# caki35/UNet-Torch

Measured on AMD Instinct MI355X. Metric: images/sec training step, 4-level U-Net 1ch→2cls 512×512, at 1/2/4/8 MI355X, higher is better.
Workload: dtype f16

## Files before the change

include/unetmi.h:

```cpp
#ifndef UNETMI_H
#define UNETMI_H
#include <stddef.h>
#include <stdint.h>

#ifdef __cplusplus
extern "C" {
#endif

typedef void* umi_stream_t;

enum { UMI_F32 = 0, UMI_F16 = 1 };
enum { UMI_OK = 0, UMI_ERR_BADARG = -1, UMI_ERR_UNSUPPORTED = -2, UMI_ERR_WORKSPACE = -3 };
enum { UMI_CONV_UPSAMPLE2 = 1,
       UMI_CONV_FORCE_GENERIC = 2,
       UMI_CONV_DGRAD_STRIDED = 4,
       UMI_CONV_ACCUMULATE = 8      };

int umi_version(void);
const char* umi_arch(void);

int umi_tune_conv3x3_impl(int impl);

int umi_pack_kn(const float* src, void* dst, int T, int K, int N, long st, long sk, long sn,
                int flip_t, int Kpad, int Npad, int dtype, umi_stream_t stream);

int umi_pack_kn8(const float* src, void* dst, int T, int K, int N, long st, long sk, long sn,
                 int flip_t, int Kpad, int Npad, int dtype, umi_stream_t stream);

int umi_conv_fwd(const void* x, int ldx, const void* tx, const void* wp, const float* bias,
                 void* y, int ldy, float* stat_part,
                 int N, int H, int W, int Ci, int Co, int R, int S, int stride, int pad,
                 int Ho, int Wo, int off_h, int off_w, int out_H, int out_W,
                 int in_dtype, int out_dtype, int flags, umi_stream_t stream);
int umi_linear_fused(const void* x, int ldx, const void* wp8, const float* bias, void* y, int ldy, long M, int Ci, int Co,
                     int epi, float p, unsigned seed, const unsigned* seed_dev, void* mask, const void* aux, int ldaux,
                     void* y2, int ldy2, int dtype, umi_stream_t stream);

int umi_conv_fwd_plan(int N, int H, int W, int Ci, int Co, int R, int S, int stride, int pad,
                      int ldx, int ldy, int in_dtype, int out_dtype, int flags, int has_bias,
                      int* layout, int* stat_rows);

int umi_bn_finalize(const float* stat_part, int rows, int C, double count,
                    const float* gamma, const float* beta, float eps, float momentum,
                    float* running_mean, float* running_var,
                    void* tx_out, float* rstd_out, umi_stream_t stream);

int umi_pool2_fwd(const void* x, int ldx, const void* tx, void* y, int ldy,
                  int N, int H, int W, int C, int dtype, umi_stream_t stream);
int umi_pool2_bwd(const void* dpool, int lddp, const void* x, int ldx, const void* tx,
                  void* da, int ldda, int accumulate,
                  int N, int H, int W, int C, int dtype, umi_stream_t stream);

size_t umi_bn_bwd_ws_bytes(long M, int C);
int umi_bn_bwd_reduce(const void* da, int ldda, const void* y, int ldy, const void* tx,
                      const float* rstd, float* sum_dz, float* sum_dzx,
                      long M, int C, int dtype, void* ws, size_t ws_bytes, umi_stream_t stream);
int umi_bn_bwd_apply(void* da, int ldda, const void* y, int ldy, const void* tx,
                     const float* rstd, const float* sum_dz, const float* sum_dzx,
                     long M, int C, int dtype, umi_stream_t stream);

int umi_conv_dgrad_bnred(const void* dy, int lddy, const void* wp8, void* da, int ldda, const void* ybn, int ldybn,
                         const void* txbn, const float* rstd, float* part, int N, int H, int W, int Ci, int Co,
                         int dtype, umi_stream_t stream);

int umi_conv_gather_bnred_rows(int N, int H, int W, int Ci, int Co, int R, int S, int stride, int pad, int Ho, int Wo,
                               int ldx, int ldy, int dtype, int flags);
int umi_conv_gather_bnred(const void* x, int ldx, const void* wp8, void* y, int ldy, const void* ybn, int ldybn,
                          const void* txbn, const float* rstd, float* part, int N, int H, int W, int Ci, int Co, int R, int S,
                          int stride, int pad, int Ho, int Wo, int dtype, int flags, umi_stream_t stream);

int umi_head_dgrad_bnred_rows(long P, int Ci, int Co, int ldda, int dtype);
int umi_head_dgrad_bnred(const void* dl, int lddl, const void* wp, void* da, int ldda, const void* ybn, int ldybn,
                         const void* txbn, const float* rstd, float* part, long P, int Ci, int Co, int dtype,
                         umi_stream_t stream);
size_t umi_head_bwd_fused_ws_bytes(long P, int Ci, int Co);
int umi_head_bwd_fused(const void* dl, int lddl, const void* wp, void* da, int ldda, const void* ybn, int ldybn,
                       const void* txbn, const float* rstd, float* part, float* dW, long s_co, long s_ci, float out_scale,
                       void* ws, size_t ws_bytes, long P, int Ci, int Co, int dtype, umi_stream_t stream);

int umi_conv3x3_fwd_act(const void* x, int ldx, const void* tx, const void* wp8, const void* out_tx, void* y, int ldy,
                        int N, int H, int W, int Ci, int Co, int dtype, umi_stream_t stream);
int umi_bn_stats_rows(long M, int C);
int umi_bn_stats(const void* x, int ldx, float* part, long M, int C, int dtype, umi_stream_t stream);
int umi_pool2_bwd_bnred_stat_rows(int N, int H, int W, int C);
int umi_pool2_bwd_bnred(const void* dpool, int lddp, const void* x, int ldx, const void* tx, const float* rstd, void* da,
                        int ldda, int accumulate, float* part, int N, int H, int W, int C, int dtype, umi_stream_t stream);
int umi_bn_bwd_from_partials(const float* part, int rows, int C, float* sum_dz, float* sum_dzx, umi_stream_t stream);

size_t umi_conv_wgrad_ws_bytes(int N, int Ho, int Wo, int Ci, int Co, int R, int S, int dtype, int flags);
int umi_conv_wgrad(const void* x, int ldx, const void* txa, const void* dy, int lddy, const void* txb,
                   float* dW, long s_co, long s_ci, long s_t, float out_scale,
                   int N, int H, int W, int Ci, int Co, int R, int S, int stride, int pad,
                   int Ho, int Wo, int dtype, int flags, void* ws, size_t ws_bytes, umi_stream_t stream);
typedef struct umi_wgrad_pending {
    const float* part;
    float* dW;
    long s_co, s_ci, s_t;
    float scale;
    int splits, RS, Ci, Co;
} umi_wgrad_pending;
int umi_conv_wgrad_deferred(const void* x, int ldx, const void* txa, const void* dy, int lddy, const void* txb,
                            float* dW, long s_co, long s_ci, long s_t, float out_scale, int N, int H, int W, int Ci, int Co,
                            int R, int S, int stride, int pad, int Ho, int Wo, int dtype, int flags, void* ws, size_t ws_bytes,
                            umi_wgrad_pending* out, umi_stream_t stream);
int umi_wgrad_reduce_group(int n, const void* items , umi_stream_t stream);
int umi_conv_wgrad_bias(const void* x, int ldx, const void* dy, int lddy, const void* txb, float* dW, long s_co, long s_ci,
                        long s_t, float* dbias, float out_scale, int N, int H, int W, int Ci, int Co, int Ho, int Wo, int dtype,
                        int flags, void* ws, size_t ws_bytes, umi_wgrad_pending* out, umi_stream_t stream);
int umi_conv_wgrad_group(int n, const void* const* x, int ldx, const void* const* dy, int lddy, float* const* dW, long s_co,
                         long s_ci, float out_scale, long M, int Ci, int Co, int dtype, umi_stream_t stream);
int umi_conv_wgrad_bnapply(const void* x, int ldx, const void* txa, const void* da, int ldda, const void* y, int ldy,
                           const void* tx_bn, const float* rstd, const float* sum_dz, const float* sum_dzx, void* dz,
                           int lddz, float* dW, long s_co, long s_ci, long s_t, float out_scale, int N, int H, int W,
                           int Ci, int Co, int R, int S, int stride, int pad, int dtype, int flags, void* ws,
                           size_t ws_bytes, umi_stream_t stream);

size_t umi_colsum_ws_bytes(long M, int C);
int umi_colsum(const void* x, int ldx, float* out, float out_scale, long M, int C, int dtype,
               void* ws, size_t ws_bytes, umi_stream_t stream);
int umi_colsum_group(int n, const void* const* xs, int ldx, float* const* outs, float out_scale, long M, int C, int dtype,
                     void* ws, size_t ws_bytes, umi_stream_t stream);

int umi_materialize_nchw(const void* x, int ldx, const void* tx, float* y_nchw,
                         int N, int H, int W, int C, int dtype, umi_stream_t stream);


int umi_wstd_fwd(const float* w, float* wstd, float* rstd, int Co, int K, float eps, umi_stream_t stream);
int umi_wstd_bwd(const float* wstd, const float* rstd, const float* g, float* dw, int Co, int K, umi_stream_t stream);
typedef struct umi_wstd_desc {
    const float* w;
    float* ws;
    float* rstd;
    long off;
    int Co, K;
    float eps;
    int blk0;
    float* dw;
} umi_wstd_desc;
int umi_wstd_fwd_multi(const void* descs, int n_desc, int total_rows, umi_stream_t stream);
int umi_wstd_bwd_multi(const void* descs, int n_desc, int total_rows, const float* g_base, float* dw_base, umi_stream_t stream);

size_t umi_gn_fwd_ws_bytes(int N, long HW, int C);
int umi_gn_fwd(const void* x, int ldx, const float* gamma, const float* beta, const void* res, int ldr, void* y, int ldy,
               float* mean, float* rstd, int relu, int N, long HW, int C, int G, float eps, int dtype,
               void* ws, size_t ws_bytes, umi_stream_t stream);
size_t umi_gn_bwd_ws_bytes(int N, long HW, int C, int G);
int umi_gn_bwd(const void* dy, int lddy, const void* y, int ldy, const void* x, int ldx, const float* mean,
               const float* rstd, const float* gamma, int relu, void* dx, int lddx, void* dres, int lddr,
               float* dgamma, float* dbeta, float out_scale, int N, long HW, int C, int G, int dtype,
               void* ws, size_t ws_bytes, float* part_out, umi_stream_t stream);
int umi_gn_param_grads_group(int n, const float* const* parts, const int* Cs, int N, float* const* dgammas,
                             float* const* dbetas, float out_scale, umi_stream_t stream);

int umi_pool3s2_fwd(const void* x, int ldx, void* y, int ldy, void* idx, int N, int H, int W, int C, int dtype,
                    umi_stream_t stream);
int umi_pool3s2_bwd(const void* dy, int lddy, const void* x, int ldx, const void* idx, void* dx, int lddx, int N, int H, int W,
                    int C, int dtype, umi_stream_t stream);

int umi_ln_fwd(const void* x, int ldx, const float* gamma, const float* beta, void* y, int ldy, float* mean, float* rstd,
               long M, int C, float eps, int dtype, umi_stream_t stream);
size_t umi_ln_bwd_ws_bytes(long M, int C);
int umi_ln_bwd(const void* dy, int lddy, const void* x, int ldx, const float* gamma, const float* mean,
               const float* rstd, void* dx, int lddx, float* dgamma, float* dbeta, float out_scale, long M, int C,
               int dtype, void* ws, size_t ws_bytes, int* rows_out, umi_stream_t stream);

int umi_elementwise(int mode, const void* x, int ldx, const void* g, int ldg, void* y, int ldy, long M, int C,
                    long bcast_rows, int dtype, umi_stream_t stream);

int umi_dropout(const void* x, int ldx, void* y, int ldy, void* mask, int backward, float p, unsigned seed, long M, int C,
                int dtype, const void* tx, const unsigned* seed_dev, umi_stream_t stream);
int umi_dropout_fused(const void* x, int ldx, void* y, int ldy, void* mask, int backward, float p, unsigned seed, long M, int C,
                      int dtype, const unsigned* seed_dev, const void* aux, int ldaux, int gelu, umi_stream_t stream);

int umi_attn_fwd(const void* q, const void* k, const void* v, int ld, void* o, int ldo, float* lse, int B, int N, int heads,
                 int D, int dtype, umi_stream_t stream);
int umi_attn_bwd(const void* q, const void* k, const void* v, int ld, const void* o, const void* dO, int ldo,
                 const float* lse, void* dq, void* dk, void* dv, int ldd, float* delta, int B, int N, int heads, int D,
                 int dtype, umi_stream_t stream);

int umi_bilinear2x(const void* x, int ldx, const void* tx, void* y, int ldy, int backward, int N, int H, int W, int C,
                   int dtype, umi_stream_t stream);

size_t umi_dice_ce_ws_bytes(int N, int C, long HW);
int umi_dice_ce_fwd(const float* logits, const void* target, int target_dtype, int N, int C, long HW, float* stats, void* ws,
                    size_t ws_bytes, umi_stream_t stream);
int umi_dice_ce_bwd(const float* logits, const void* target, int target_dtype, const float* stats, const float* gout, int N,
                    int C, long HW, float* dlogits, umi_stream_t stream);

size_t umi_hdt_ws_bytes(int B, int H, int W);
int umi_hdt_fwd(const float* pred, const float* target, int B, int C, int H, int W, float alpha, float* D, float* fields,
                float* loss, void* ws, size_t ws_bytes, umi_stream_t stream);
int umi_hdt_bwd(const float* pred, const float* target, const float* D, const float* gout, int B, int C, int H, int W,
                float* dpred, umi_stream_t stream);

size_t umi_binloss_ws_bytes(int B, int C, long HW);
int umi_dice_bce_fwd(const float* pred, const float* target, int B, long HW, double* stats, float* loss, void* ws,
                     size_t ws_bytes, umi_stream_t stream);
int umi_dice_bce_bwd(const float* pred, const float* target, const double* stats, const float* gout, int B, long HW,
                     float* dpred, umi_stream_t stream);
int umi_tversky_fwd(const float* pred, const void* target, int target_dtype, int B, int C, long HW, float alpha, float beta,
                    double* stats, float* loss, void* ws, size_t ws_bytes, umi_stream_t stream);
int umi_tversky_bwd(const float* pred, const void* target, int target_dtype, const double* stats, const float* gout, int B,
                    int C, long HW, float alpha, float beta, float* dpred, umi_stream_t stream);

size_t umi_topk_loss_ws_bytes(long N);
int umi_topk_loss_fwd(const float* pred, const float* target, long N, long k, int mode, unsigned char* mask, float* loss,
                      void* ws, size_t ws_bytes, umi_stream_t stream);
int umi_topk_loss_bwd(const float* pred, const float* target, const unsigned char* mask, const float* gout, long N, long k,
                      float* dpred, umi_stream_t stream);

size_t umi_mt_ratio_ws_bytes(int B, long HW);
size_t umi_mt_ratio_stats_len(int B);
int umi_mt_ratio_fwd(const float* o1, const float* o2, const float* l1, const float* l2, int B, long HW, int gate,
                     const float* gate_dev, double* stats, float* loss, float* loss1, float* loss2, float* ratio, void* ws, size_t ws_bytes,
                     umi_stream_t stream);
int umi_mt_ratio_bwd(const float* o1, const float* o2, const float* l1, const float* l2, const double* stats,
                     const float* gout, int B, long HW, float* d1, float* d2, umi_stream_t stream);

typedef struct umi_optim_desc {
    float* p;
    const float* g;
    float* s0;
// ... 95 lines not shown
```

unet-torch_amd/csrc/conv1x1_mfma.hip:

```cpp
#include "common.h"
#include <stdlib.h>
#include <string.h>

typedef _Float16 half8 __attribute__((ext_vector_type(8)));
typedef _Float16 half4 __attribute__((ext_vector_type(4)));
typedef float floatx16 __attribute__((ext_vector_type(16)));
typedef float floatx4 __attribute__((ext_vector_type(4)));
typedef unsigned u32x4 __attribute__((ext_vector_type(4)));

struct UmiLinearEpi { int mode; float p; unsigned seed; const unsigned* seed_dev; void* mask; const void* aux; int ldaux; void* y2; int ldy2;
                      const void* bn_tx; const float* bn_rstd; float* bn_part; };

namespace {

constexpr int OUT_UPS_TAPS_MAX = 49;

constexpr int CK = 64;
constexpr int ROWB = 160;

struct Geo {
    int h, w;
    int Hs, Ws, soy, sox;
    int Hd, Wd, doy, dox;
    int S, stride, pad, frac;
// ... 268 lines not shown
            tdx = (tap & 1) + geo.dox;
        }
        constexpr int NPS = P / PSTEP;
        half8 ybv[NPS];
        if (geo.epi == 3 && !OUT_UPS) {
#pragma unroll
            for (int k = 0; k < NPS; ++k) {
                const int p = p0 + k * PSTEP;
                if (m0 + p < M && col_ok) {
                    const int2 pi = dense ? make_int2(0, 0) : pixinfo[p];
                    const long drow = dense ? (m0 + p) : ((long)pi.x * geo.Hd + (pi.y >> 16)) * geo.Wd + (pi.y & 0xffff);
                    ybv[k] = *reinterpret_cast<const half8*>(geo.aux + drow * geo.ldaux + cop);
                }
            }
        }
#pragma unroll
        for (int k = 0; k < NPS; ++k) {
            const int p = p0 + k * PSTEP;
            if (m0 + p >= M || !col_ok) break;
            const int2 pi = dense ? make_int2(0, 0) : pixinfo[p];
            int yy = pi.y >> 16, xx = pi.y & 0xffff;
            if (OUT_UPS) {
                yy = 2 * yy + tdy;
                xx = 2 * xx + tdx;
                if (yy < 0 || yy >= geo.Hd || xx < 0 || xx >= geo.Wd) continue;
            }
            uint4 v = *reinterpret_cast<const uint4*>(smem + p * ERS + j * 16);
            half_t* dst = dense ? y + (m0 + p) * ldy + co : y + ((long)((long)pi.x * geo.Hd + yy) * geo.Wd + xx) * ldy + co;
            if (geo.accum) {
                const half8 o = *reinterpret_cast<const half8*>(dst);
                v = __builtin_bit_cast(uint4, (half8)(o + __builtin_bit_cast(half8, v)));
            }
            if (geo.epi == 1 || geo.epi == 2) {
                const long e0 = (m0 + p) * (long)Ntot_ + cop;
                const unsigned seed = geo.seed + (geo.seed_dev ? geo.seed_dev[0] * 0x9E3779B9u : 0u);
                const float scale = 1.f / (1.f - geo.drop_p);
                const half8 xv = __builtin_bit_cast(half8, v);
                half8 av, o;
                if (geo.epi == 2) av = *reinterpret_cast<const half8*>(geo.aux + (m0 + p) * geo.ldaux + cop);
                unsigned long long mk = 0;
#pragma unroll
                for (int jj = 0; jj < 8; ++jj) {
                    const long e = e0 + jj;
                    const float u = (c1_hash32((unsigned)e, seed ^ (unsigned)(e >> 32)) >> 8) * (1.f / 16777216.f);
                    const unsigned k = u >= geo.drop_p;
                    mk |= (unsigned long long)k << (8 * jj);
                    float f = (float)xv[jj];
                    if (geo.epi == 1) f = c1_gelu(f);
                    f = k ? f * scale : 0.f;
                    if (geo.epi == 2) f += (float)av[jj];
                    o[jj] = (half_t)f;
                }
                *reinterpret_cast<unsigned long long*>(geo.mask + e0) = mk;
                if (geo.epi == 1) *reinterpret_cast<half8*>(geo.y2 + (m0 + p) * geo.ldy2 + cop) = o;
                else v = __builtin_bit_cast(uint4, o);
            }
#ifdef UMI_X_NOSTORE
            if (v.x == 0x12345678u)
#endif
            *reinterpret_cast<uint4*>(dst) = v;
            if (geo.epi == 3 && !OUT_UPS) {
                const half8 yv = ybv[k];
                const half8 hv = __builtin_bit_cast(half8, v);
#pragma unroll
                for (int jj = 0; jj < 8; ++jj) {
                    const float yy_ = (float)yv[jj];
                    const float dz = umi_tx_pre(yy_, bt[jj]) > bt[jj].w ? (float)hv[jj] : 0.f;
                    bs[jj] += dz;
                    bq[jj] = fmaf(dz, (yy_ - bt[jj].x) * brs[jj], bq[jj]);
                }
            }
        }
        if (geo.epi == 3) {
            __syncthreads();
            float* rs_ = reinterpret_cast<float*>(smem);
#pragma unroll
            for (int jj = 0; jj < 8; ++jj) {
                rs_[(0 * PSTEP + p0) * BN + j * 8 + jj] = bs[jj];
                rs_[(1 * PSTEP + p0) * BN + j * 8 + jj] = bq[jj];
            }
            __syncthreads();
            if (tid < 2 * BN) {
                const int which = tid / BN, cc = tid % BN;
                float a = 0.f;
#pragma unroll 8
                for (int k = 0; k < PSTEP; ++k) a += rs_[(which * PSTEP + k) * BN + cc];
                if (c0 + cc < Ntot_) geo.bn_part[((m0 / P) * 2 + which) * Ntot_ + c0 + cc] = a;
            }
        }
    }
}

template <int P, int BN>
int launch(bool s2d, bool ups, const void* x, int ldx, const void* tx, const void* wp8, const float* bias, void* y,
           int ldy, long M, int Kc, int Nc, int Ntot, int ntaps, Geo geo, hipStream_t s) {
    const int n_co = (Ntot + BN - 1) / BN;
    const long nblk = ((M + P - 1) / P) * n_co;
    dim3 grid((unsigned)((nblk + 7) / 8 * 8)), block(256);
#define GO(S2D, UPS, HT)                                                                                          \
    hipLaunchKernelGGL((conv1x1_mfma_kernel<P, BN, S2D, UPS, HT>), grid, block, 0, s, (const half_t*)x, ldx,      \
                       (const float4*)tx, (const half_t*)wp8, bias, (half_t*)y, ldy, M, Kc, Nc, n_co, ntaps, geo, nblk)
    if (s2d) { if (tx) GO(true, false, true); else GO(true, false, false); }
    else if (ups) { if (tx) GO(false, true, true); else GO(false, true, false); }
    else { if (tx) GO(false, false, true); else GO(false, false, false); }
#undef GO
    UMI_LAUNCH_CHECK();
    return UMI_OK;
}

}

int umi_conv1x1_mode(int R, int S, int stride, int pad, int flags) {
    if (flags & UMI_CONV_UPSAMPLE2) return (R == 2 && S == 2) ? 1 : -1;
    if (R * S > 49 || pad < 0 || pad >= 1 << 20) return -1;
    if (flags & UMI_CONV_DGRAD_STRIDED) return stride >= 1 ? 2 : -1;
    if (R == 1 && S == 1 && stride == 1 && pad == 0) return 0;
    if (stride >= 2) return 2;
    return -1;
}

bool umi_conv1x1_mfma_ok(int Ci, int Co, int R, int S, int stride, int pad, int ldx, int ldy, int in_dtype,
                         int out_dtype, int flags) {
    if (flags & UMI_CONV_FORCE_GENERIC) return false;
    if (in_dtype != UMI_F16 || out_dtype != UMI_F16) return false;
    const int mode = umi_conv1x1_mode(R, S, stride, pad, flags);
    if (mode < 0) return false;
    if (ldx % 8 || ldy % 8) return false;
    if ((long)(OUT_UPS_TAPS_MAX) * Ci * Co * 2 >= 0x7FFFFFF0L) return false;
    if (mode == 0) return Ci % 8 == 0 && Co % 8 == 0 && Ci >= 16 && Co >= 16;
    if (Ci % 64 || Co % 64) return false;
    return true;
}

static void c1_pick_tile(long M, int Ntot, int* P, int* BN) {
    const bool bn128 = Ntot % 128 == 0;
    const long want = 300;
    const long b_256_128 = ((M + 255) / 256) * (Ntot / 128), b_128_128 = ((M + 127) / 128) * (Ntot / 128);
    const long b_256_64 = ((M + 255) / 256) * (Ntot / 64);
    if (const char* e = getenv("UMI_C1_TILE")) {
        const int p_ = atoi(e), bn_ = strchr(e, 'x') ? atoi(strchr(e, 'x') + 1) : 0;
        if ((p_ == 256 || p_ == 128) && ((bn_ == 128 && bn128) || bn_ == 64)) { *P = p_; *BN = bn_; return; }
    }
    if (bn128 && b_256_128 >= want) { *P = 256; *BN = 128; return; }
    if (b_256_64 >= want) { *P = 256; *BN = 64; return; }
    if (bn128 && b_128_128 >= want) { *P = 128; *BN = 128; return; }
    *P = 128; *BN = 64;
}
int umi_conv1x1_bnred_rows(long M, int Ntot) {
    int P, BN;
    c1_pick_tile(M, Ntot, &P, &BN);
    return (int)((M + P - 1) / P);
}

int umi_conv1x1_mfma(const void* x, int ldx, const void* tx, const void* wp8, const float* bias, void* y, int ldy,
                     int N, int H, int W, int Ci, int Co, int R, int S, int stride, int pad, int Ho, int Wo, int off_h,
                     int off_w, int out_H, int out_W, int flags, hipStream_t s, const UmiLinearEpi* epi) {
    const int mode = umi_conv1x1_mode(R, S, stride, pad, flags);
    if (epi && epi->mode && epi->mode != 3 && (mode != 0 || (flags & UMI_CONV_ACCUMULATE) || Co % 8)) return UMI_ERR_UNSUPPORTED;
    if (epi && epi->mode == 3 && (mode == 1 || Co % 8)) return UMI_ERR_UNSUPPORTED;
    Geo geo;
    long M;
    int Kc = Ci, Nc = Co, Ntot = Co, ntaps = 1;
    if (mode == 0) {
        geo = Geo{H, W, H, W, 0, 0, H, W, 0, 0, 1, 1, 0, 0};
        M = (long)N * H * W;
    } else if (mode == 1) {
        geo = Geo{H, W, H, W, 0, 0, out_H, out_W, off_h, off_w, 1, 1, 0, 0};
        M = (long)N * H * W;
        Ntot = 4 * Co;
    } else {
        geo = Geo{Ho, Wo, H, W, 0, 0, Ho, Wo, 0, 0, S, stride, pad, (flags & UMI_CONV_DGRAD_STRIDED) ? 1 : 0};
        M = (long)N * Ho * Wo;
        ntaps = R * S;
    }
    if (mode != 0 && 2L * H * W * ldx * 2 >= 0x7FFFFFF0L) return UMI_ERR_UNSUPPORTED;
    geo.accum = (flags & UMI_CONV_ACCUMULATE) ? 1 : 0;
    geo.epi = 0; geo.drop_p = 0.f; geo.seed = 0; geo.seed_dev = nullptr; geo.mask = nullptr; geo.aux = nullptr; geo.ldaux = 0;
    geo.y2 = nullptr; geo.ldy2 = 0; geo.bn_tx = nullptr; geo.bn_rstd = nullptr; geo.bn_part = nullptr;
    if (epi && epi->mode) {
        geo.epi = epi->mode; geo.drop_p = epi->p; geo.seed = epi->seed; geo.seed_dev = epi->seed_dev;
        geo.mask = (unsigned char*)epi->mask; geo.aux = (const half_t*)epi->aux; geo.ldaux = epi->ldaux;
        geo.y2 = (half_t*)epi->y2; geo.ldy2 = epi->ldy2;
        geo.bn_tx = (const float4*)epi->bn_tx; geo.bn_rstd = epi->bn_rstd; geo.bn_part = epi->bn_part;
    }
#define GO(P_, BN_) return launch<P_, BN_>(mode == 2, mode == 1, x, ldx, tx, wp8, bias, y, ldy, M, Kc, Nc, Ntot, ntaps, geo, s)
    int tp, tbn;
    c1_pick_tile(M, Ntot, &tp, &tbn);
    if (tp == 256 && tbn == 128) GO(256, 128);
    if (tp == 256) GO(256, 64);
    if (tbn == 128) GO(128, 128);
    GO(128, 64);
#undef GO
}
```

unet-torch_amd/umi/lib.py:

```python
import ctypes
import os
from ctypes import c_char_p, c_double, c_float, c_int, c_long, c_size_t, c_uint, c_void_p

from . import build as _build

UMI_F32, UMI_F16 = 0, 1
CONV_UPSAMPLE2, CONV_FORCE_GENERIC, CONV_DGRAD_STRIDED, CONV_ACCUMULATE = 1, 2, 4, 8

_ERR = {-1: "UMI_ERR_BADARG", -2: "UMI_ERR_UNSUPPORTED", -3: "UMI_ERR_WORKSPACE"}


def _load():
    alt = os.environ.get("UMI_LIB_OVERRIDE")
    if alt:
        if not os.path.exists(alt):
            raise RuntimeError(f"UMI_LIB_OVERRIDE={alt} does not exist")
        return ctypes.CDLL(alt)
    path = _build.LIB
    if not os.path.exists(path) or (_build.stale() and os.path.exists(_build.HIPCC)):
        if not os.path.exists(_build.HIPCC):
            raise RuntimeError(
                f"libunetmi.so not found at {path} and hipcc is unavailable: the HIP extension is "
                "required, there is no CPU fallback (run `python __graft_entry__.py build`).")
        _build.build_lib()
    return ctypes.CDLL(path)


_lib = _load()

SIGNATURES = {
    "umi_version": (c_int, []),
    "umi_arch": (c_char_p, []),
    "umi_tune_conv3x3_impl": (c_int, [c_int]),
    "umi_zoom_cubic_ws_bytes": (c_size_t, [c_int, c_int, c_int]),
    "umi_zoom_cubic_hwc": (c_int, [c_void_p, c_int, c_void_p, c_int, c_int, c_int, c_int, c_int, c_void_p, c_size_t, c_void_p]),
    "umi_linear_fused": (c_int, [c_void_p, c_int, c_void_p, c_void_p, c_void_p, c_int, c_long, c_int, c_int, c_int, c_float,
                                 c_uint, c_void_p, c_void_p, c_void_p, c_int, c_void_p, c_int, c_int, c_void_p]),
    "umi_pack_kn": (c_int, [c_void_p, c_void_p, c_int, c_int, c_int, c_long, c_long, c_long, c_int, c_int, c_int,
                            c_int, c_void_p]),
    "umi_pack_kn8": (c_int, [c_void_p, c_void_p, c_int, c_int, c_int, c_long, c_long, c_long, c_int, c_int, c_int,
                             c_int, c_void_p]),
    "umi_conv_fwd": (c_int, [c_void_p, c_int, c_void_p, c_void_p, c_void_p, c_void_p, c_int, c_void_p,
                             c_int, c_int, c_int, c_int, c_int, c_int, c_int, c_int, c_int,
                             c_int, c_int, c_int, c_int, c_int, c_int, c_int, c_int, c_int, c_void_p]),
    "umi_conv_fwd_plan": (c_int, [c_int] * 15 + [c_void_p, c_void_p]),
    "umi_bn_finalize": (c_int, [c_void_p, c_int, c_int, c_double, c_void_p, c_void_p, c_float, c_float,
                                c_void_p, c_void_p, c_void_p, c_void_p, c_void_p]),
    "umi_pool2_fwd": (c_int, [c_void_p, c_int, c_void_p, c_void_p, c_int, c_int, c_int, c_int, c_int, c_int,
                              c_void_p]),
    "umi_pool2_bwd": (c_int, [c_void_p, c_int, c_void_p, c_int, c_void_p, c_void_p, c_int, c_int,
                              c_int, c_int, c_int, c_int, c_int, c_void_p]),
    "umi_bn_bwd_ws_bytes": (c_size_t, [c_long, c_int]),
    "umi_bn_bwd_reduce": (c_int, [c_void_p, c_int, c_void_p, c_int, c_void_p, c_void_p, c_void_p, c_void_p,
                                  c_long, c_int, c_int, c_void_p, c_size_t, c_void_p]),
    "umi_bn_bwd_apply": (c_int, [c_void_p, c_int, c_void_p, c_int, c_void_p, c_void_p, c_void_p, c_void_p,
                                 c_long, c_int, c_int, c_void_p]),
    "umi_conv_wgrad_ws_bytes": (c_size_t, [c_int] * 9),
    "umi_conv_wgrad": (c_int, [c_void_p, c_int, c_void_p, c_void_p, c_int, c_void_p, c_void_p,
                               c_long, c_long, c_long, c_float,
                               c_int, c_int, c_int, c_int, c_int, c_int, c_int, c_int, c_int, c_int, c_int,
                               c_int, c_int, c_void_p, c_size_t, c_void_p]),
    "umi_conv_wgrad_deferred": (c_int, [c_void_p, c_int, c_void_p, c_void_p, c_int, c_void_p, c_void_p,
                                        c_long, c_long, c_long, c_float,
                                        c_int, c_int, c_int, c_int, c_int, c_int, c_int, c_int, c_int, c_int, c_int,
                                        c_int, c_int, c_void_p, c_size_t, c_void_p, c_void_p]),
    "umi_wgrad_reduce_group": (c_int, [c_int, c_void_p, c_void_p]),
    "umi_conv_wgrad_group": (c_int, [c_int, c_void_p, c_int, c_void_p, c_int, c_void_p, c_long, c_long, c_float, c_long,
                                     c_int, c_int, c_int, c_void_p]),
    "umi_conv_wgrad_bnapply": (c_int, [c_void_p, c_int, c_void_p, c_void_p, c_int, c_void_p, c_int, c_void_p, c_void_p, c_void_p,
                                       c_void_p, c_void_p, c_int, c_void_p, c_long, c_long, c_long, c_float,
                                       c_int, c_int, c_int, c_int, c_int, c_int, c_int, c_int, c_int, c_int, c_int,
                                       c_void_p, c_size_t, c_void_p]),
    "umi_colsum_ws_bytes": (c_size_t, [c_long, c_int]),
    "umi_colsum_group": (c_int, [c_int, c_void_p, c_int, c_void_p, c_float, c_long, c_int, c_int, c_void_p, c_size_t, c_void_p]),
    "umi_materialize_nchw": (c_int, [c_void_p, c_int, c_void_p, c_void_p, c_int, c_int, c_int, c_int, c_int, c_void_p]),
    "umi_wstd_fwd": (c_int, [c_void_p, c_void_p, c_void_p, c_int, c_int, c_float, c_void_p]),
    "umi_wstd_bwd": (c_int, [c_void_p, c_void_p, c_void_p, c_void_p, c_int, c_int, c_void_p]),
    "umi_wstd_fwd_multi": (c_int, [c_void_p, c_int, c_int, c_void_p]),
    "umi_wstd_bwd_multi": (c_int, [c_void_p, c_int, c_int, c_void_p, c_void_p, c_void_p]),
    "umi_gn_fwd": (c_int, [c_void_p, c_int, c_void_p, c_void_p, c_void_p, c_int, c_void_p, c_int, c_void_p, c_void_p, c_int,
                           c_int, c_long, c_int, c_int, c_float, c_int, c_void_p, c_size_t, c_void_p]),
    "umi_gn_fwd_ws_bytes": (c_size_t, [c_int, c_long, c_int]),
    "umi_gn_bwd_ws_bytes": (c_size_t, [c_int, c_long, c_int, c_int]),
    "umi_gn_bwd": (c_int, [c_void_p, c_int, c_void_p, c_int, c_void_p, c_int, c_void_p, c_void_p, c_void_p, c_int,
                           c_void_p, c_int, c_void_p, c_int, c_void_p, c_void_p, c_float, c_int, c_long, c_int, c_int, c_int,
                           c_void_p, c_size_t, c_void_p, c_void_p]),
    "umi_gn_param_grads_group": (c_int, [c_int, c_void_p, c_void_p, c_int, c_void_p, c_void_p, c_float, c_void_p]),
    "umi_pool3s2_fwd": (c_int, [c_void_p, c_int, c_void_p, c_int, c_void_p, c_int, c_int, c_int, c_int, c_int, c_void_p]),
    "umi_pool3s2_bwd": (c_int, [c_void_p, c_int, c_void_p, c_int, c_void_p, c_void_p, c_int, c_int, c_int, c_int, c_int, c_int,
                                c_void_p]),
    "umi_ln_fwd": (c_int, [c_void_p, c_int, c_void_p, c_void_p, c_void_p, c_int, c_void_p, c_void_p, c_long, c_int, c_float,
                           c_int, c_void_p]),
    "umi_ln_bwd_ws_bytes": (c_size_t, [c_long, c_int]),
    "umi_ln_bwd": (c_int, [c_void_p, c_int, c_void_p, c_int, c_void_p, c_void_p, c_void_p, c_void_p, c_int, c_void_p, c_void_p,
                           c_float, c_long, c_int, c_int, c_void_p, c_size_t, c_void_p, c_void_p]),
    "umi_elementwise": (c_int, [c_int, c_void_p, c_int, c_void_p, c_int, c_void_p, c_int, c_long, c_int, c_long, c_int, c_void_p]),
    "umi_dropout": (c_int, [c_void_p, c_int, c_void_p, c_int, c_void_p, c_int, c_float, ctypes.c_uint, c_long, c_int, c_int,
                            c_void_p, c_void_p, c_void_p]),
    "umi_dropout_fused": (c_int, [c_void_p, c_int, c_void_p, c_int, c_void_p, c_int, c_float, ctypes.c_uint, c_long, c_int, c_int,
                                  c_void_p, c_void_p, c_int, c_int, c_void_p]),
    "umi_attn_fwd": (c_int, [c_void_p, c_void_p, c_void_p, c_int, c_void_p, c_int, c_void_p, c_int, c_int, c_int, c_int, c_int,
                             c_void_p]),
    "umi_attn_bwd": (c_int, [c_void_p, c_void_p, c_void_p, c_int, c_void_p, c_void_p, c_int, c_void_p, c_void_p, c_void_p,
                             c_void_p, c_int, c_void_p, c_int, c_int, c_int, c_int, c_int, c_void_p]),
    "umi_bilinear2x": (c_int, [c_void_p, c_int, c_void_p, c_void_p, c_int, c_int, c_int, c_int, c_int, c_int, c_int, c_void_p]),
    "umi_colsum": (c_int, [c_void_p, c_int, c_void_p, c_float, c_long, c_int, c_int, c_void_p, c_size_t, c_void_p]),
    "umi_conv3x3_fwd_act": (c_int, [c_void_p, c_int, c_void_p, c_void_p, c_void_p, c_void_p, c_int, c_int, c_int, c_int, c_int,
                                    c_int, c_int, c_void_p]),
    "umi_conv_dgrad_bnred": (c_int, [c_void_p, c_int, c_void_p, c_void_p, c_int, c_void_p, c_int, c_void_p, c_void_p, c_void_p,
                                     c_int, c_int, c_int, c_int, c_int, c_int, c_void_p]),
    "umi_conv_wgrad_bias": (c_int, [c_void_p, c_int, c_void_p, c_int, c_void_p, c_void_p, c_long, c_long, c_long, c_void_p, c_float]
                            + [c_int] * 9 + [c_void_p, c_size_t, c_void_p, c_void_p]),
    "umi_conv_gather_bnred_rows": (c_int, [c_int] * 15),
    "umi_conv_gather_bnred": (c_int, [c_void_p, c_int, c_void_p, c_void_p, c_int, c_void_p, c_int, c_void_p, c_void_p, c_void_p]
                              + [c_int] * 13 + [c_void_p]),
    "umi_head_bwd_fused_ws_bytes": (c_size_t, [c_long, c_int, c_int]),
    "umi_head_bwd_fused": (c_int, [c_void_p, c_int, c_void_p, c_void_p, c_int, c_void_p, c_int, c_void_p, c_void_p, c_void_p,
                                   c_void_p, c_long, c_long, c_float, c_void_p, c_size_t, c_long, c_int, c_int, c_int, c_void_p]),
    "umi_head_dgrad_bnred_rows": (c_int, [c_long, c_int, c_int, c_int, c_int]),
    "umi_head_dgrad_bnred": (c_int, [c_void_p, c_int, c_void_p, c_void_p, c_int, c_void_p, c_int, c_void_p, c_void_p, c_void_p,
                                     c_long, c_int, c_int, c_int, c_void_p]),
    "umi_bn_bwd_from_partials": (c_int, [c_void_p, c_int, c_int, c_void_p, c_void_p, c_void_p]),
    "umi_bn_stats_rows": (c_int, [c_long, c_int]),
    "umi_bn_stats": (c_int, [c_void_p, c_int, c_void_p, c_long, c_int, c_int, c_void_p]),
    "umi_pool2_bwd_bnred_stat_rows": (c_int, [c_int, c_int, c_int, c_int]),
    "umi_pool2_bwd_bnred": (c_int, [c_void_p, c_int, c_void_p, c_int, c_void_p, c_void_p, c_void_p, c_int, c_int, c_void_p,
                                    c_int, c_int, c_int, c_int, c_int, c_void_p]),
    "umi_dice_ce_ws_bytes": (c_size_t, [c_int, c_int, c_long]),
    "umi_dice_ce_fwd": (c_int, [c_void_p, c_void_p, c_int, c_int, c_int, c_long, c_void_p, c_void_p, c_size_t, c_void_p]),
    "umi_dice_ce_bwd": (c_int, [c_void_p, c_void_p, c_int, c_void_p, c_void_p, c_int, c_int, c_long, c_void_p, c_void_p]),
    "umi_hdt_ws_bytes": (c_size_t, [c_int, c_int, c_int]),
    "umi_hdt_fwd": (c_int, [c_void_p, c_void_p, c_int, c_int, c_int, c_int, c_float, c_void_p, c_void_p, c_void_p, c_void_p,
                            c_size_t, c_void_p]),
    "umi_hdt_bwd": (c_int, [c_void_p, c_void_p, c_void_p, c_void_p, c_int, c_int, c_int, c_int, c_void_p, c_void_p]),
    "umi_binloss_ws_bytes": (c_size_t, [c_int, c_int, c_long]),
    "umi_dice_bce_fwd": (c_int, [c_void_p, c_void_p, c_int, c_long, c_void_p, c_void_p, c_void_p, c_size_t, c_void_p]),
    "umi_dice_bce_bwd": (c_int, [c_void_p, c_void_p, c_void_p, c_void_p, c_int, c_long, c_void_p, c_void_p]),
    "umi_tversky_fwd": (c_int, [c_void_p, c_void_p, c_int, c_int, c_int, c_long, c_float, c_float, c_void_p, c_void_p,
                                c_void_p, c_size_t, c_void_p]),
    "umi_tversky_bwd": (c_int, [c_void_p, c_void_p, c_int, c_void_p, c_void_p, c_int, c_int, c_long, c_float, c_float,
                                c_void_p, c_void_p]),
    "umi_topk_loss_ws_bytes": (c_size_t, [c_long]),
    "umi_topk_loss_fwd": (c_int, [c_void_p, c_void_p, c_long, c_long, c_int, c_void_p, c_void_p, c_void_p, c_size_t,
                                  c_void_p]),
    "umi_topk_loss_bwd": (c_int, [c_void_p, c_void_p, c_void_p, c_void_p, c_long, c_long, c_void_p, c_void_p]),
    "umi_mt_ratio_ws_bytes": (c_size_t, [c_int, c_long]),
    "umi_mt_ratio_stats_len": (c_size_t, [c_int]),
    "umi_mt_ratio_fwd": (c_int, [c_void_p, c_void_p, c_void_p, c_void_p, c_int, c_long, c_int, c_void_p, c_void_p, c_void_p,
                                 c_void_p, c_void_p, c_void_p, c_void_p, c_size_t, c_void_p]),
    "umi_mt_ratio_bwd": (c_int, [c_void_p, c_void_p, c_void_p, c_void_p, c_void_p, c_void_p, c_int, c_long, c_void_p,
                                 c_void_p, c_void_p]),
    "umi_optim_block_elems": (c_int, []),
    "umi_table_upload": (c_int, [c_void_p, c_void_p, c_size_t, c_void_p]),
    "umi_optim_sgd_multi": (c_int, [c_void_p, c_int, c_int, c_double, c_double, c_double, c_double, c_int, c_int, c_void_p]),
    "umi_optim_adam_multi": (c_int, [c_void_p, c_int, c_int, c_double, c_double, c_double, c_double, c_double, c_double,
                                     c_void_p]),
    "umi_optim_hyper_bytes": (c_size_t, []),
    "umi_optim_hyper_pre": (c_int, [c_void_p, c_int, c_void_p]),
    "umi_optim_hyper_poly": (c_int, [c_void_p, c_void_p]),
    "umi_optim_sgd_multi_dev": (c_int, [c_void_p, c_int, c_int, c_void_p, c_double, c_double, c_double, c_int, c_int, c_void_p]),
    "umi_optim_adam_multi_dev": (c_int, [c_void_p, c_int, c_int, c_void_p, c_double, c_double, c_double, c_double, c_void_p]),
    "umi_pack_block_elems": (c_int, []),
    "umi_pack_kn_multi": (c_int, [c_void_p, c_int, c_int, c_int, c_void_p]),
    "umi_add2_relu_fwd": (c_int, [c_void_p, c_int, c_void_p, c_void_p, c_int, c_void_p, c_void_p, c_int, c_long, c_int, c_int,
                                  c_void_p]),
    "umi_add2_relu_bwd": (c_int, [c_void_p, c_int, c_void_p, c_int, c_void_p, c_int, c_void_p, c_int, c_long, c_int, c_int,
                                  c_void_p]),
    "umi_gate_fwd": (c_int, [c_void_p, c_int, c_void_p, c_void_p, c_void_p, c_void_p, c_int, c_long, c_int, c_int, c_void_p]),
    "umi_gate_bwd": (c_int, [c_void_p, c_int, c_void_p, c_int, c_void_p, c_void_p, c_void_p, c_void_p, c_int, c_void_p,
                             c_long, c_int, c_int, c_void_p]),
    "umi_znorm_ws_bytes": (c_size_t, []),
    "umi_znorm_hwc": (c_int, [c_void_p, c_int, c_void_p, c_long, c_int, c_int, c_void_p, c_size_t, c_void_p]),
    "umi_argmax_mask": (c_int, [c_void_p, c_void_p, c_int, c_int, c_long, c_void_p]),
    "umi_binary_mask": (c_int, [c_void_p, c_void_p, c_long, c_void_p]),
    "umi_zoom_nearest": (c_int, [c_void_p, c_int, c_void_p, c_int, c_int, c_int, c_int, c_int, c_void_p]),
    "umi_sum_trunc_ws_bytes": (c_size_t, [c_int]),
    "umi_sum_trunc": (c_int, [c_void_p, c_void_p, c_int, c_long, c_void_p, c_size_t, c_void_p]),
    "umi_components_ws_bytes": (c_size_t, [c_int, c_int, c_int]),
    "umi_components_cap": (c_int, [c_int, c_int]),
    "umi_count_components": (c_int, [c_void_p, c_void_p, c_int, c_int, c_int, c_void_p, c_size_t, c_void_p]),
    "umi_label_components": (c_int, [c_void_p, c_void_p, c_void_p, c_void_p, c_void_p, c_void_p, c_int, c_int, c_int, c_void_p,
                                     c_size_t, c_void_p]),
    "umi_match_max_dots": (c_int, []),
    "umi_dot_lists_ws_bytes": (c_size_t, [c_int, c_int, c_int]),
    "umi_dot_lists": (c_int, [c_void_p, c_int, c_void_p, c_void_p, c_int, c_int, c_int, c_int, c_void_p, c_size_t, c_void_p]),
    "umi_component_centers": (c_int, [c_void_p, c_void_p, c_void_p, c_void_p, c_void_p, c_int, c_int, c_void_p]),
    "umi_crowd_match": (c_int, [c_void_p, c_void_p, c_int, c_void_p, c_void_p, c_int, c_void_p, c_size_t, c_void_p, c_int,
                                c_void_p, c_int, c_void_p, c_int, c_void_p]),
    "umi_distance_match_ws_bytes": (c_size_t, [c_int, c_int]),
    "umi_distance_match": (c_int, [c_void_p, c_void_p, c_int, c_void_p, c_void_p, c_int, ctypes.c_longlong, c_void_p, c_int,
                                   c_void_p, c_size_t, c_void_p]),
    "umi_grid_sums": (c_int, [c_void_p, c_int, c_void_p, c_int, c_int, c_int, c_int, c_void_p]),
    "umi_scatter_centers": (c_int, [c_void_p, c_void_p, c_int, c_void_p, c_int, c_int, c_int, c_void_p]),
    "umi_class_components_ws_bytes": (c_size_t, [c_int, c_int, c_int, c_int]),
    "umi_count_class_components": (c_int, [c_void_p, c_void_p, c_int, c_int, c_int, c_int, c_void_p, c_size_t, c_void_p]),
    "umi_label_class_components": (c_int, [c_void_p, c_void_p, c_void_p, c_void_p, c_void_p, c_void_p, c_void_p, c_void_p, c_int,
                                           c_int, c_int, c_int, c_int, c_void_p, c_size_t, c_void_p]),
    "umi_split_classes": (c_int, [c_void_p, c_void_p, c_int, c_int, c_int, c_int, c_void_p]),
    "umi_class_center_lists": (c_int, [c_void_p, c_void_p, c_void_p, c_void_p, c_void_p, c_void_p, c_void_p, c_int, c_int, c_int,
                                       c_void_p]),
}

for _name, (_res, _args) in SIGNATURES.items():
    _fn = getattr(_lib, _name)
    _fn.restype = _res
    _fn.argtypes = _args


def check(status: int, what: str):
    if status != 0:
        raise RuntimeError(f"libunetmi: {what} failed with "
                           f"{_ERR.get(status, 'hipError_t ' + str(status))}")


def fn(name):
    return getattr(_lib, name)


lib = _lib
```

Measured before the change: 761.5.

## Add persistent streaming MFMA kernel for 2x2 transposed-conv upsample forward

Adds a persistent kernel for the stride-2 2x2 transposed convolution forward. Each block keeps one output-channel weight tile resident in LDS and walks pixel tiles in stripes. Activation loads for the next tile are prefetched into registers while the current tile runs MFMA, and results are staged through LDS so output stores go out as coalesced 16-byte buffer stores. It is routed automatically for Kc of 128 or 256 with no epilogue, and can be turned off with an environment variable. The aim is to cut repeated weight loads and launch/tail overhead in the upsampling convs, at the cost of extra code and occupancy assumptions (a hardcoded 256 CUs and XCD-swizzled block mapping).

```diff
diff --git a/include/unetmi.h b/include/unetmi.h
--- a/include/unetmi.h
+++ b/include/unetmi.h
@@ -68,6 +68,8 @@
 int umi_conv_gather_bnred(const void* x, int ldx, const void* wp8, void* y, int ldy, const void* ybn, int ldybn,
                           const void* txbn, const float* rstd, float* part, int N, int H, int W, int Ci, int Co, int R, int S,
                           int stride, int pad, int Ho, int Wo, int dtype, int flags, umi_stream_t stream);
+
+int umi_convt_stream_route(int mode, long M, int Kc, int Nc, int flags, int epi_mode);
 
 int umi_head_dgrad_bnred_rows(long P, int Ci, int Co, int ldda, int dtype);
 int umi_head_dgrad_bnred(const void* dl, int lddl, const void* wp, void* da, int ldda, const void* ybn, int ldybn,
diff --git a/unet-torch_amd/csrc/conv1x1_mfma.hip b/unet-torch_amd/csrc/conv1x1_mfma.hip
--- a/unet-torch_amd/csrc/conv1x1_mfma.hip
+++ b/unet-torch_amd/csrc/conv1x1_mfma.hip
@@ -444,6 +444,9 @@
     return (int)((M + P - 1) / P);
 }
 
+int umi_convt_stream_fwd(const void* x, int ldx, const void* tx, const void* wp8, const float* bias, void* y, int ldy, int N,
+                         int h, int w, int Kc, int Nc, hipStream_t s);
+
 int umi_conv1x1_mfma(const void* x, int ldx, const void* tx, const void* wp8, const float* bias, void* y, int ldy,
                      int N, int H, int W, int Ci, int Co, int R, int S, int stride, int pad, int Ho, int Wo, int off_h,
                      int off_w, int out_H, int out_W, int flags, hipStream_t s, const UmiLinearEpi* epi) {
@@ -475,6 +478,11 @@
         geo.y2 = (half_t*)epi->y2; geo.ldy2 = epi->ldy2;
         geo.bn_tx = (const float4*)epi->bn_tx; geo.bn_rstd = epi->bn_rstd; geo.bn_part = epi->bn_part;
     }
+    if (mode == 1 && off_h == 0 && off_w == 0 && out_H == 2 * H && out_W == 2 * W &&
+        umi_convt_stream_route(mode, M, Kc, Nc, flags, geo.epi)) {
+        const int rc = umi_convt_stream_fwd(x, ldx, tx, wp8, bias, y, ldy, N, H, W, Kc, Nc, s);
+        if (rc != UMI_ERR_UNSUPPORTED) return rc;
+    }
 #define GO(P_, BN_) return launch<P_, BN_>(mode == 2, mode == 1, x, ldx, tx, wp8, bias, y, ldy, M, Kc, Nc, Ntot, ntaps, geo, s)
     int tp, tbn;
     c1_pick_tile(M, Ntot, &tp, &tbn);
diff --git a/unet-torch_amd/csrc/convT_stream_mfma.hip b/unet-torch_amd/csrc/convT_stream_mfma.hip
--- /dev/null
+++ b/unet-torch_amd/csrc/convT_stream_mfma.hip
@@ -0,0 +1,241 @@
+#include "common.h"
+#include <stdlib.h>
+
+typedef _Float16 half8 __attribute__((ext_vector_type(8)));
+typedef _Float16 half4 __attribute__((ext_vector_type(4)));
+typedef float floatx4 __attribute__((ext_vector_type(4)));
+typedef unsigned u32x4 __attribute__((ext_vector_type(4)));
+
+namespace {
+
+constexpr int SP = 128;
+constexpr int SBN = 128;
+constexpr int ERS = SBN * 2 + 16;
+constexpr unsigned OOB = 0x7FFFFFFFu;
+constexpr int CUS = 256;
+
+struct StreamArgs {
+    long M;
+    int h, w;
+    int ldx, ldy;
+    int Nc;
+    int n_co;
+    int npt;
+    int stripes;
+    long ybytes;
+};
+
+constexpr int lds_bytes(int KC) { return 2 * SP * (KC * 2 + 32) + 4 * SP * 4; }
+
+template <int KC, bool HAS_TX>
+__global__ __launch_bounds__(256, KC == 128 ? 2 : 1) void convT_stream_fwd_kernel(
+    const half_t* __restrict__ x, const float4* __restrict__ tx, const half_t* __restrict__ wp8,
+    const float* __restrict__ bias, half_t* __restrict__ y, StreamArgs g) {
+    constexpr int RS = KC * 2 + 32;
+    constexpr int WB = SBN * RS, XB = SP * RS;
+    constexpr int PPRX = KC / 8;
+    constexpr int RPP = 256 / PPRX;
+    constexpr int NLD = SP / RPP;
+    constexpr int NST = SP * (SBN / 8) / 256;
+    constexpr int D = KC == 128 ? 1 : 2;
+    static_assert(SP * ERS <= XB, "the output tile aliases the x tile");
+    extern __shared__ __attribute__((aligned(16))) unsigned char smem[];
+    unsigned char* const ws = smem;
+    unsigned char* const xs = smem + WB;
+    unsigned* const pixo = reinterpret_cast<unsigned*>(smem + WB + XB);
+
+    const int tid = threadIdx.x, lane = tid & 63, wave = tid >> 6;
+    const int wn = wave & 1, wm = wave >> 1;
+    const int lrow = lane & 15, lgrp = lane >> 4;
+    const int per_xcd = (int)gridDim.x >> 3;
+    const int gid = (int)(blockIdx.x & 7) * per_xcd + (int)(blockIdx.x >> 3);
+    const int cb = gid % g.n_co, stripe = gid / g.n_co;
+    if (stripe >= g.npt) return;
+    const int c0 = cb * SBN;
+    const int ntl = (g.npt - stripe + g.stripes - 1) / g.stripes;
+
+#pragma unroll
+    for (int k = 0; k < SBN * PPRX / 256; ++k) {
+        const int idx = tid + 256 * k;
+        const int c = idx % SBN, s8 = idx / SBN;
+        const int cop = c0 + c, tap = cop / g.Nc, co = cop - tap * g.Nc;
+        *reinterpret_cast<u32x4*>(ws + c * RS + s8 * 16) =
+            *reinterpret_cast<const u32x4*>(wp8 + ((long)(tap * PPRX + s8) * g.Nc + co) * 8);
+    }
+    const int pc = tid % PPRX, pr = tid / PPRX;
+    float4 t[8];
+    if (HAS_TX) {
+#pragma unroll
+        for (int j = 0; j < 8; ++j) t[j] = tx[pc * 8 + j];
+    }
+    float bv[4][4];
+#pragma unroll
+    for (int ct = 0; ct < 4; ++ct) {
+        const float4 b4 = bias ? *reinterpret_cast<const float4*>(bias + (c0 + wn * 64 + ct * 16 + lgrp * 4) % g.Nc)
+                               : make_float4(0.f, 0.f, 0.f, 0.f);
+        bv[ct][0] = b4.x; bv[ct][1] = b4.y; bv[ct][2] = b4.z; bv[ct][3] = b4.w;
+    }
+    const int sj = tid % (SBN / 8), sp0 = tid / (SBN / 8);
+    unsigned tapoff;
+    {
+        const int cop = c0 + sj * 8, tap = cop / g.Nc, co = cop - tap * g.Nc;
+        tapoff = (unsigned)((((tap >> 1) * 2 * g.w + (tap & 1)) * g.ldy + co) * 2);
+    }
+    const unsigned xo0 = (unsigned)((pr * g.ldx + pc * 8) * 2), xstep = (unsigned)(RPP * g.ldx * 2);
+    const unsigned hw = (unsigned)(g.h * g.w);
+    const long yimg = (long)4 * hw * g.ldy * 2;
+
+    u32x4 xraw[D][NLD];
+    __amdgpu_buffer_rsrc_t yrs = __builtin_amdgcn_make_buffer_rsrc((void*)y, 0, 0, 0x00020000);
+#define UMI_ISSUE(i_, S_)                                                                                           \
+    do {                                                                                                          \
+        const int ti = stripe + (i_) * g.stripes;                                                                 \
+        const long m0 = (long)ti * SP;                                                                            \
+        const bool live = (i_) < ntl;                                                                             \
+        const long left = live ? g.M - m0 : 0;                                                                    \
+        const __amdgpu_buffer_rsrc_t xrs = __builtin_amdgcn_make_buffer_rsrc(                                     \
+            (void*)(x + (live ? m0 * g.ldx : 0)), 0, (int)((left < SP ? left : SP) * g.ldx * 2), 0x00020000);    \
+        _Pragma("unroll") for (int k = 0; k < NLD; ++k)                                                           \
+            xraw[S_][k] = __builtin_bit_cast(u32x4, __builtin_amdgcn_raw_buffer_load_b128(xrs, xo0 + k * xstep, 0, 0)); \
+        if (tid < SP) {                                                                                           \
+            unsigned o = 0x80000000u;                                                                             \
+            if (live && m0 + tid < g.M) {                                                                         \
+                const unsigned n0 = (unsigned)m0 / hw, m = (unsigned)m0 + tid;                                    \
+                const unsigned n = m / hw, r = m - n * hw;                                                        \
+                const unsigned yy = r / (unsigned)g.w, xx = r - yy * (unsigned)g.w;                               \
+                o = (unsigned)((((long)(n - n0) * 2 * g.h + 2 * yy) * 2 * g.w + 2 * xx) * g.ldy * 2);            \
+            }                                                                                                     \
+            pixo[((i_) & 3) * SP + tid] = o;                                                                      \
+        }                                                                                                         \
+    } while (0)
+
+    UMI_ISSUE(0, 0);
+#pragma unroll
+    for (int k = 0; k < NST; ++k) __builtin_amdgcn_raw_buffer_store_b128(u32x4{0u, 0u, 0u, 0u}, yrs, OOB - 16u * k, 0, 0);
+    if (D == 2) {
+        UMI_ISSUE(1, D - 1);
+#pragma unroll
+        for (int k = 0; k < NST; ++k) __builtin_amdgcn_raw_buffer_store_b128(u32x4{0u, 0u, 0u, 0u}, yrs, OOB - 16u * (NST + k), 0, 0);
+    }
+    const int b_base = (wm * 64 + lrow) * RS + lgrp * 16;
+    const int a_base = (wn * 64 + lrow) * RS + lgrp * 16;
+
+#define UMI_TILE(i_, S_)                                                                                          \
+    do {                                                                                                          \
+        const int it = (i_);                                                                                      \
+                                                 \
+        _Pragma("unroll") for (int k = 0; k < NLD; ++k) {                                                         \
+            u32x4 v = xraw[S_][k];                                                                                \
+            if (HAS_TX) v = __builtin_bit_cast(u32x4, umi_tx8(__builtin_bit_cast(half8, v), t));                  \
+            *reinterpret_cast<u32x4*>(xs + (pr + RPP * k) * RS + pc * 16) = v;                                    \
+        }                                                                                                         \
+        __syncthreads();                                                                                          \
+        UMI_ISSUE(it + D, S_);                               \
+        {                                                                                                         \
+            const bool live = it < ntl;                                                                           \
+            const long m0 = (long)(stripe + it * g.stripes) * SP;                                                 \
+            const long n0 = live ? (long)((unsigned)m0 / hw) : 0;                                                 \
+            const long left = live ? g.ybytes - n0 * yimg : 0;                                                    \
+            yrs = __builtin_amdgcn_make_buffer_rsrc((void*)((char*)y + n0 * yimg), 0,                             \
+                                                    (int)(left > 0x7FFFFFF0L ? 0x7FFFFFF0L : left), 0x00020000); \
+        }                                                                                                         \
+        floatx4 acc[4][4];                                                                                        \
+        _Pragma("unroll") for (int a = 0; a < 4; ++a)                                                             \
+            _Pragma("unroll") for (int b = 0; b < 4; ++b)                                                         \
+                _Pragma("unroll") for (int r = 0; r < 4; ++r) acc[a][b][r] = 0.f;                                 \
+        __builtin_amdgcn_s_setprio(3);                                                                            \
+        _Pragma("unroll") for (int ks = 0; ks < KC / 32; ++ks) {                                                  \
+            half8 af[4];                                                                                          \
+            _Pragma("unroll") for (int ct = 0; ct < 4; ++ct)                                                      \
+                af[ct] = *reinterpret_cast<const half8*>(ws + a_base + ct * 16 * RS + ks * 64);                   \
+            _Pragma("unroll") for (int ph = 0; ph < 2; ++ph) {                                                    \
+                half8 bf[2];                                                                                      \
+                _Pragma("unroll") for (int q = 0; q < 2; ++q)                                                     \
+                    bf[q] = *reinterpret_cast<const half8*>(xs + b_base + (ph * 2 + q) * 16 * RS + ks * 64);      \
+                _Pragma("unroll") for (int ct = 0; ct < 4; ++ct)                                                  \
+                    _Pragma("unroll") for (int q = 0; q < 2; ++q)                                                 \
+                        acc[ct][ph * 2 + q] =                                                                     \
+                            __builtin_amdgcn_mfma_f32_16x16x32_f16(af[ct], bf[q], acc[ct][ph * 2 + q], 0, 0, 0);  \
+            }                                                                                                     \
+        }                                                                                                         \
+        __builtin_amdgcn_s_setprio(0);                                                                            \
+        __syncthreads();                                                  \
+                         \
+        _Pragma("unroll") for (int ct = 0; ct < 4; ++ct) {                                                        \
+            const int col = wn * 64 + ct * 16 + lgrp * 4;                                                         \
+            _Pragma("unroll") for (int pt = 0; pt < 4; ++pt) {                                                    \
+                const int pix = wm * 64 + pt * 16 + lrow;                                                         \
+                half4 hv;                                                                                         \
+                _Pragma("unroll") for (int j = 0; j < 4; ++j) hv[j] = (half_t)(acc[ct][pt][j] + bv[ct][j]);       \
+                *reinterpret_cast<half4*>(xs + pix * ERS + col * 2) = hv;                                         \
+            }                                                                                                     \
+        }                                                                                                         \
+        __syncthreads();                                                                                          \
+        _Pragma("unroll") for (int k = 0; k < NST; ++k) {                                                         \
+            const int p = sp0 + k * (256 / (SBN / 8));                                                            \
+            const unsigned po = pixo[(it & 3) * SP + p];                                                          \
+            const u32x4 v = *reinterpret_cast<const u32x4*>(xs + p * ERS + sj * 16);                              \
+            __builtin_amdgcn_raw_buffer_store_b128(v, yrs, (po & 0x80000000u) ? OOB : po + tapoff, 0, 0);         \
+        }                                                                                                         \
+        __syncthreads();                                   \
+    } while (0)
+
+    for (int i = 0; i < ntl; i += D) {
+        UMI_TILE(i, 0);
+        if (D == 2) UMI_TILE(i + 1, D - 1);
+    }
+#undef UMI_TILE
+#undef UMI_ISSUE
+}
+
+template <int KC>
+int launch_stream(const void* x, const void* tx, const void* wp8, const float* bias, void* y, const StreamArgs& g, hipStream_t s) {
+    constexpr int dyn = lds_bytes(KC);
+    static const int attr_rc = [] {
+        int a = (int)hipFuncSetAttribute((const void*)convT_stream_fwd_kernel<KC, true>, hipFuncAttributeMaxDynamicSharedMemorySize, dyn);
+        int b = (int)hipFuncSetAttribute((const void*)convT_stream_fwd_kernel<KC, false>, hipFuncAttributeMaxDynamicSharedMemorySize, dyn);
+        return a ? a : b;
+    }();
+    if (attr_rc) return attr_rc;
+    dim3 grid((unsigned)(g.stripes * g.n_co)), block(256);
+    if (tx)
+        hipLaunchKernelGGL((convT_stream_fwd_kernel<KC, true>), grid, block, dyn, s, (const half_t*)x, (const float4*)tx,
+                           (const half_t*)wp8, bias, (half_t*)y, g);
+    else
+        hipLaunchKernelGGL((convT_stream_fwd_kernel<KC, false>), grid, block, dyn, s, (const half_t*)x, (const float4*)tx,
+                           (const half_t*)wp8, bias, (half_t*)y, g);
+    UMI_LAUNCH_CHECK();
+    return UMI_OK;
+}
+
+}
+
+extern "C" int umi_convt_stream_route(int mode, long M, int Kc, int Nc, int flags, int epi_mode) {
+    if (const char* e = getenv("UMI_CONVT_STREAM"))
+        if (e[0] == '0' && e[1] == 0) return 0;
+    if (mode != 1 || epi_mode != 0) return 0;
+    if (flags & (UMI_CONV_ACCUMULATE | UMI_CONV_FORCE_GENERIC | UMI_CONV_DGRAD_STRIDED)) return 0;
+    if (Kc != 128 && Kc != 256) return 0;
+    if (Nc < 32 || (4 * Nc) % SBN) return 0;
+    if (M <= 0 || M >= 0x7FFFFFFFL - SP) return 0;
+    return 1;
+}
+
+int umi_convt_stream_fwd(const void* x, int ldx, const void* tx, const void* wp8, const float* bias, void* y, int ldy, int N,
+                         int h, int w, int Kc, int Nc, hipStream_t s) {
+    StreamArgs g;
+    g.M = (long)N * h * w;
+    g.h = h; g.w = w; g.ldx = ldx; g.ldy = ldy; g.Nc = Nc;
+    g.n_co = 4 * Nc / SBN;
+    g.npt = (int)((g.M + SP - 1) / SP);
+    const long yimg = (long)4 * h * w * ldy * 2;
+    if (((SP - 1) / ((long)h * w) + 2) * yimg >= 0x7FFFFFF0L || (long)SP * ldx * 2 >= 0x7FFFFFF0L) return UMI_ERR_UNSUPPORTED;
+    g.ybytes = (long)N * yimg;
+    const int per_cu = 2 * lds_bytes(Kc) <= 160 * 1024 ? 2 : 1;
+    int stripes = CUS * per_cu / g.n_co / 8 * 8;
+    if (stripes < 8) stripes = 8;
+    const int need = (g.npt + 7) / 8 * 8;
+    g.stripes = need < stripes ? need : stripes;
+    if (Kc == 128) return launch_stream<128>(x, tx, wp8, bias, y, g, s);
+    return launch_stream<256>(x, tx, wp8, bias, y, g, s);
+}
diff --git a/unet-torch_amd/umi/lib.py b/unet-torch_amd/umi/lib.py
--- a/unet-torch_amd/umi/lib.py
+++ b/unet-torch_amd/umi/lib.py
@@ -114,6 +114,7 @@
     "umi_conv_gather_bnred_rows": (c_int, [c_int] * 15),
     "umi_conv_gather_bnred": (c_int, [c_void_p, c_int, c_void_p, c_void_p, c_int, c_void_p, c_int, c_void_p, c_void_p, c_void_p]
                               + [c_int] * 13 + [c_void_p]),
+    "umi_convt_stream_route": (c_int, [c_int, c_long, c_int, c_int, c_int, c_int]),
     "umi_head_bwd_fused_ws_bytes": (c_size_t, [c_long, c_int, c_int]),
     "umi_head_bwd_fused": (c_int, [c_void_p, c_int, c_void_p, c_void_p, c_int, c_void_p, c_int, c_void_p, c_void_p, c_void_p,
                                    c_void_p, c_long, c_long, c_float, c_void_p, c_size_t, c_long, c_int, c_int, c_int, c_void_p]),
```

New measurement: 764.8, median of 6. About the same (+0.4%).
